# volume-em/empanada-napari

Hardware: AMD Instinct MI355X
Metric: EM tiles/sec (1024^2 fp16) (higher is better)
Workload: dtype f16

## Files before the change

empanada-napari_amd/build.py:

```python
import os
import shutil
import subprocess
import sys

HERE = os.path.dirname(os.path.abspath(__file__))
CSRC = os.path.join(HERE, 'csrc')
OBJ = os.path.join(CSRC, '_obj')
LIBDIR = os.path.join(HERE, 'lib')
LIB = os.path.join(LIBDIR, 'libempanada_hip.so')
ARCH = 'gfx950'

COMMON = ['--offload-arch=' + ARCH, '-O3', '-std=c++17', '-fPIC', '-fvisibility=hidden',
          '-Wall', '-Wno-unused-function', '-Wno-unused-result']
PER_FILE = {
    'postprocess.hip': ['-ffp-contract=off', '-fhip-fp32-correctly-rounded-divide-sqrt'],
}
SOURCES = ['abi.hip', 'conv_igemm.hip', 'layers.hip', 'pointrend.hip', 'postprocess.hip', 'pdl_net.hip', 'sparse.hip',
           'sepconv.hip', 'sepconv_precise.hip', 'conv_igemm256.hip', 'conv_igemm_s64.hip', 'conv3x3c64.hip', 'stem.hip', 'matcher.hip', 'ref32.hip', 'conv16x3.hip', 'conv_igemm_grouped.hip', 'conv16x3p.hip', 'sepconv_x3.hip', 'overlap.hip', 'labels.hip', 'morph.hip']
INCLUDES = {'conv_igemm_grouped.hip': ['conv_igemm.hip']}


def _hipcc():
    for cand in (shutil.which('hipcc'), '/opt/rocm/bin/hipcc'):
        if cand and os.path.exists(cand):
            return cand
    raise RuntimeError('hipcc not found: the HIP engine cannot be built (no CPU fallback exists)')


def _newest_header():
    hs = [os.path.join(CSRC, f) for f in os.listdir(CSRC) if f.endswith('.h')]
    hs.append(os.path.join(HERE, '..', 'include', 'empanada_hip.h'))
    return max(os.path.getmtime(h) for h in hs)


def build_all(verbose=False, force=False):
    os.makedirs(OBJ, exist_ok=True)
    os.makedirs(LIBDIR, exist_ok=True)
    hipcc = _hipcc()
    hdr = _newest_header()
    objs, rebuilt = [], False
    procs = []
    for src in SOURCES:
        s = os.path.join(CSRC, src)
        o = os.path.join(OBJ, src.replace('.hip', '.o'))
        objs.append(o)
        dep = max([os.path.getmtime(s), hdr] + [os.path.getmtime(os.path.join(CSRC, d)) for d in INCLUDES.get(src, [])])
        if force or not os.path.exists(o) or os.path.getmtime(o) < dep:
            cmd = [hipcc] + COMMON + PER_FILE.get(src, []) + ['-c', s, '-o', o]
            if verbose:
                print(' '.join(cmd), flush=True)
            procs.append((src, subprocess.Popen(cmd, stdout=subprocess.PIPE, stderr=subprocess.STDOUT)))
# ... 19 lines not shown
```

empanada-napari_amd/csrc/abi.hip:

```cpp
#include <stdarg.h>

#include <map>
#include <mutex>
#include <utility>
#include <vector>

#include "common.h"

namespace emp {

static thread_local char g_err[1024] = "no error";

void set_error(const char* fmt, ...) {
  va_list ap;
  va_start(ap, fmt);
  vsnprintf(g_err, sizeof(g_err), fmt, ap);
  va_end(ap);
}

const void* zero_page() {
  static void* page = nullptr;
  static std::once_flag once;
  std::call_once(once, [] {
    if (hipMalloc(&page, 2048) != hipSuccess) { page = nullptr; return; }
// ... 83 lines not shown
  p.out = d_out; p.out_ld = out_ld;
  p.N = N; p.H = H; p.W = W; p.Cin = Cin; p.Cout = Cout; p.KH = KH; p.KW = KW; p.stride = stride; p.pad = pad; p.dil = dil;
  p.Ho = (H + 2 * pad - dil * (KH - 1) - 1) / stride + 1;
  p.Wo = (W + 2 * pad - dil * (KW - 1) - 1) / stride + 1;
  EMP_REQUIRE(p.Ho > 0 && p.Wo > 0 && out_ld >= Cout && (d_res == nullptr || res_ld >= Cout), "conv2d_f32: bad output geometry");
  p.act = act;
  return launch_conv32(p, (hipStream_t)stream);
}

int emp_conv2d_nhwc_f16x3(const float* d_in, int N, int H, int W, int Cin, int in_ld, const float* d_w, const float* d_bias,
                          const float* d_bias_n, const float* d_res, int res_ld, float* d_out, int out_ld, int Cout, int KH,
                          int KW, int stride, int pad, int dil, int act, int groups, int cin_g, void* stream) {
  EMP_REQUIRE(d_in && d_w && d_out, "conv2d_f16x3: null pointer");
  EMP_REQUIRE(N > 0 && H > 0 && W > 0 && KH > 0 && KW > 0 && stride > 0 && dil > 0 && pad >= 0 && groups >= 1, "conv2d_f16x3: bad geometry");
  Conv32 p{};
  p.in = d_in; p.in_ld = in_ld; p.w = d_w; p.bias = d_bias; p.bias_n = d_bias_n; p.res = d_res; p.res_ld = res_ld;
  p.out = d_out; p.out_ld = out_ld;
  p.N = N; p.H = H; p.W = W; p.Cin = Cin; p.Cout = Cout; p.KH = KH; p.KW = KW; p.stride = stride; p.pad = pad; p.dil = dil;
  p.Ho = (H + 2 * pad - dil * (KH - 1) - 1) / stride + 1;
  p.Wo = (W + 2 * pad - dil * (KW - 1) - 1) / stride + 1;
  EMP_REQUIRE(p.Ho > 0 && p.Wo > 0 && out_ld >= groups * Cout && (d_res == nullptr || res_ld >= Cout), "conv2d_f16x3: bad output geometry");
  p.act = act;
  p.x3 = 1;
  if (groups > 1) { p.groups = groups; p.cin_g = cin_g; }
  return launch_conv32(p, (hipStream_t)stream);
}

int emp_conv2d_nhwc_f16x3_ex(const float* d_in, int N, int H, int W, int Cin, int in_ld, const float* d_w, const float* d_bias,
                             const float* d_bias_n, const float* d_res, int res_ld, void* d_out, int out_ld, int out_fmt, int Cout, int KH,
                             int KW, int stride, int pad, int dil, int act, int wmode, const float* d_in2, int H2, int W2, int Cin2,
                             int in2_ld, int stride2, const float* d_head_w, const float* d_head_b, int head_c, float* d_head_out,
                             void* stream) {
  EMP_REQUIRE(d_in && d_w && (d_out || d_head_w), "conv2d_f16x3_ex: null pointer");
  EMP_REQUIRE(N > 0 && H > 0 && W > 0 && KH > 0 && KW > 0 && stride > 0 && dil > 0 && pad >= 0 && wmode >= 0 && (wmode & 3) <= 2 && wmode < 8,
              "conv2d_f16x3_ex: bad geometry (wmode 0 fp32 weights, 1 split pairs, 2 pairs + LDS-DMA image; + 4: split-K allowed)");
  const bool ksplit = (wmode & 4) != 0;
  wmode &= 3;
  hipStream_t s = (hipStream_t)stream;
  Conv32 p{};
  p.in = d_in; p.in_ld = in_ld; p.w = d_w; p.bias = d_bias; p.bias_n = d_bias_n; p.res = d_res; p.res_ld = res_ld;
  p.out = (float*)d_out; p.out_ld = out_ld; p.out_fmt = out_fmt;
  p.N = N; p.H = H; p.W = W; p.Cin = Cin; p.Cout = Cout; p.KH = KH; p.KW = KW; p.stride = stride; p.pad = pad; p.dil = dil;
  p.Ho = (H + 2 * pad - dil * (KH - 1) - 1) / stride + 1;
  p.Wo = (W + 2 * pad - dil * (KW - 1) - 1) / stride + 1;
  EMP_REQUIRE(p.Ho > 0 && p.Wo > 0 && (d_head_w || out_ld >= Cout) && (d_res == nullptr || res_ld >= Cout), "conv2d_f16x3_ex: bad output geometry");
  p.act = act;
  p.x3 = 1;
  if (d_in2) { p.in2 = d_in2; p.in2_ld = in2_ld; p.Cin2 = Cin2; p.H2 = H2; p.W2 = W2; p.stride2 = stride2; }
  const int64_t Krow = (int64_t)KH * KW * Cin + (d_in2 ? Cin2 : 0);
  std::vector<void*> tmp;
  auto cleanup = [&]() { for (void* q : tmp) (void)hipFree(q); };
  int rc = EMP_OK;
  if (wmode >= 1) {
    void* d = nullptr;
    if (hipMalloc(&d, (size_t)Cout * Krow * sizeof(uint32_t)) != hipSuccess) { cleanup(); set_error("conv2d_f16x3_ex: out of memory"); return EMP_ERR_NOMEM; }
    tmp.push_back(d);
    p.wpair = (const uint32_t*)d;
    rc = launch_split_pairs(d_w, (uint32_t*)d, (int64_t)Cout * Krow, s);
  }
  if (!rc && wmode == 2 && !d_in2) {
    const int64_t ih = x3_weight_image_halfs(Cout, (int)Krow, Cin);
    if (ih > 0) {
      void* d = nullptr;
      if (hipMalloc(&d, (size_t)ih * sizeof(half_t)) != hipSuccess) { cleanup(); set_error("conv2d_f16x3_ex: out of memory"); return EMP_ERR_NOMEM; }
      tmp.push_back(d);
      p.wimg = (const half_t*)d;
      rc = launch_x3_weight_image(d_w, (half_t*)d, Cout, (int)Krow, s);
    }
  }
  if (!rc && ksplit && !d_head_w && !d_in2) {
    void* d = nullptr;
    if (hipMalloc(&d, (size_t)X3_KPART_BYTES) != hipSuccess) { cleanup(); set_error("conv2d_f16x3_ex: out of memory"); return EMP_ERR_NOMEM; }
    tmp.push_back(d);
    p.kpart = (float*)d; p.kpart_bytes = X3_KPART_BYTES;
  }
  const int64_t MP = (int64_t)N * p.Ho * p.Wo;
  const int tiles = conv16x3_cout_tiles(Cout);
  if (!rc && d_head_w) {
    EMP_REQUIRE(d_head_out && head_c >= 1 && head_c <= 4, "conv2d_f16x3_ex: the fused head writes (N, head_c, Ho * Wo) floats, head_c <= 4");
    void* d = nullptr;
    if (hipMalloc(&d, (size_t)tiles * MP * head_c * sizeof(float)) != hipSuccess) { cleanup(); set_error("conv2d_f16x3_ex: out of memory"); return EMP_ERR_NOMEM; }
    tmp.push_back(d);
    p.head_w = d_head_w; p.head_part = (float*)d; p.head_c = head_c;
    if (!p.out) { p.out = d_head_out; p.out_ld = Cout; }
  }
  if (!rc) rc = launch_conv32(p, s);
  if (!rc && d_head_w) rc = launch_head_finish_f32(p.head_part, tiles, N, p.Ho * p.Wo, head_c, d_head_b, d_head_out, s);
  hipError_t e = hipStreamSynchronize(s);
  cleanup();
  if (!rc && e != hipSuccess) { set_error("conv2d_f16x3_ex: %s", hipGetErrorString(e)); return EMP_ERR_HIP; }
  return rc;
}

int emp_sepconv_x3_pack(const float* d_dw, const float* d_pw, int ks, int C, int Cout, float* d_dw_packed, void* d_pw_packed, void* stream) {
  int rc = launch_sepx3_pack_dw(d_dw, ks, C, C, d_dw_packed, (hipStream_t)stream);
  if (rc) return rc;
  return launch_sepx3_pack_pw(d_pw, C, C, Cout, (half_t*)d_pw_packed, (hipStream_t)stream);
}
int emp_sepconv_x3_nhwc_f32(const float* d_in, int N, int H, int W, int C, int in_ld, const float* d_dw_packed, const void* d_pw_packed,
                            const float* d_bias, int Cout, int act, float* d_out, int out_ld, const float* d_head_w, const float* d_head_b,
// ... 357 lines not shown
```

empanada-napari_amd/csrc/common.h:

```cpp
#pragma once
#include <hip/hip_runtime.h>
#include <stdint.h>
#include <stdio.h>
#include <string>

#include "../../include/empanada_hip.h"

typedef _Float16 half_t;
typedef _Float16 f16x8 __attribute__((ext_vector_type(8)));
typedef _Float16 f16x4 __attribute__((ext_vector_type(4)));
typedef _Float16 f16x2 __attribute__((ext_vector_type(2)));
typedef float f32x4 __attribute__((ext_vector_type(4)));

namespace emp {

void set_error(const char* fmt, ...);

#define EMP_CHECK_HIP(expr)                                                        \
  do {                                                                             \
    hipError_t _e = (expr);                                                        \
    if (_e != hipSuccess) {                                                        \
      emp::set_error("%s:%d: %s -> %s", __FILE__, __LINE__, #expr, hipGetErrorString(_e)); \
      return EMP_ERR_HIP;                                                          \
    }                                                                              \
// ... 94 lines not shown
int launch_sepconvp_pack_pw(const float* w, int pw_ld, int C, int Cout, half_t* packed, hipStream_t s, int wsplit = 0);
int launch_sepconvp_pack_dw(const float* w, int ks, int C, float* packed, hipStream_t s);
int launch_sepconvp(const half_t* in, int N, int H, int W, int C, int in_ld, const float* dww_packed, const half_t* pww_packed,
                    const float* bias, int Cout, int act, half_t* out, int out_ld, const float* head_w,
                    const float* head_b, int head_c, float* hout, int64_t plane, const half_t* zero, hipStream_t s,
                    int ks = 5, int wsplit = 0);
int launch_head1x1(const half_t* in, int N, int P, int K, int in_ld, const float* w, const float* b, int C,
                   float* out, int64_t plane_size, const int32_t* scatter_idx, hipStream_t s);
int launch_bilinear_ac_f32_nchw(const float* in, int NC, int h, int w, float* out, int scale, hipStream_t s);
int launch_zero(void* p, size_t bytes, hipStream_t s);

struct Conv32 {
  const float* in; int in_ld;
  const float* w; const float* bias; const float* bias_n;
  const float* res; int res_ld;
  float* out; int out_ld;
  int N, H, W, Cin, Cout, KH, KW, stride, pad, dil, Ho, Wo;
  int act;
  int ps_cout;
  int groups;
  int cin_g;
  int x3;
  const float* in2; int in2_ld, Cin2, H2, W2, stride2;
  const float* head_w; float* head_part; int head_c;
  int x3_mt, x3_nt, x3_mtx;
  const float* zero;
  const uint32_t* wpair;
  const half_t* wimg;
  int in_fmt, out_fmt, res_fmt;
  const half_t* wimgp;
  float* out2; int out2_ld, split2;
  int x3p_kg;
  float* kpart; int64_t kpart_bytes; int ksplit, x3_ksteps;
};
constexpr int64_t X3_KPART_BYTES = 64ll << 20;
int launch_conv32(const Conv32& p, hipStream_t s);
int launch_conv16x3(const Conv32& p, hipStream_t s);
int launch_split_pairs(const float* w, uint32_t* out, int64_t n, hipStream_t s);
int64_t x3_weight_image_halfs(int Cout, int K, int Cin);
int launch_x3_weight_image(const float* w, half_t* out, int Cout, int K, hipStream_t s);
bool conv16x3p_supported(const Conv32& p);
int launch_conv16x3p(const Conv32& p, hipStream_t s);
int64_t x3p_image_halfs(int Cout, int K);
int x3p_kgroup(int KT, int Cin);
int launch_x3p_pack(const float* w, half_t* out, int Cout, int K, hipStream_t s, int KT = 0, int Cin = 0, int kg = 0);
int launch_hl32_from_f32(const float* in, half_t* out, int64_t rows, int C, int in_ld, int out_ld, hipStream_t s);
int launch_hl32_to_f32(const half_t* in, float* out, int64_t rows, int C, int in_ld, int out_ld, hipStream_t s);
int launch_avgpool_hl32(const half_t* in, int N, int HW, int C, int in_ld, float* out, hipStream_t s);
bool sepconv_x3_supported(int C, int Cout, int head_c, int ks);
int64_t sepx3_pw_halfs(int C, int Cout);
int launch_sepx3_pack_pw(const float* w, int pw_ld, int C, int Cout, half_t* packed, hipStream_t s);
int launch_sepx3_pack_dw(const float* w , int ks, int C, int ld, float* packed, hipStream_t s);
int launch_sepconv_x3(const float* in, int N, int H, int W, int C, int in_ld, const float* dww, const half_t* pww, const float* bias,
                      int Cout, int act, float* out, int out_ld, const float* head_w, const float* head_b, int head_c, float* hout,
                      int64_t plane, hipStream_t s, int ks = 5);
int conv16x3_cout_tiles(int Cout);
int launch_head_finish_f32(const float* part, int tiles, int N, int P, int C, const float* b, float* out, hipStream_t s);
int launch_stem3x3s2_f32(const void* img, int dtype, float sub, float mul, int N, int H, int W, int vh, int vw,
                         const float* w , const float* b, int C, float* out, int out_ld, hipStream_t s);
int launch_gate_mul_f32(float* x, int x_ld, const float* g, int g_ld, int64_t rows, int C, hipStream_t s);
int launch_stem7x7_f32(const void* img, int dtype, float sub, float mul, int N, int H, int W, int vh, int vw,
                       const float* w , const float* b , float* out, hipStream_t s);
int launch_maxpool3x3s2_f32(const float* in, int N, int H, int W, int C, float* out, hipStream_t s);
int launch_dwconv_f32(const float* in, int N, int H, int W, int C, int in_ld, const float* w , int K, float* out,
                      int out_ld, hipStream_t s);
int launch_bilinear_ac_f32_nhwc(const float* in, int N, int h, int w, int C, int in_ld, float* out, int H, int W, int out_ld,
                                hipStream_t s);
int launch_avgpool_f32(const float* in, int N, int HW, int C, int in_ld, float* out, hipStream_t s);
int launch_fuse_combine_f32(const float* a, const float* b, const float* c, float ca, float cb, float cc, int mode, int N,
                            int H, int W, int C, float* out, hipStream_t s);
int launch_head1x1_f32(const float* in, int N, int P, int K, int in_ld, const float* w, const float* b, int C, float* out,
                       int64_t plane_size, const int32_t* scatter_idx, hipStream_t s);
int launch_point_features_f32(const float* feat, int N, int fh, int fw, int C, int feat_ld, const float* coarse, int ncls,
// ... 26 lines not shown
```

empanada-napari_amd/csrc/conv16x3.hip:

```cpp
#include <type_traits>

#include "common.h"

namespace emp {
namespace {

constexpr int X_BK = 32, X_LD = 32;

template <int ACT>
__device__ __forceinline__ float x_act(float x) {
  if (ACT == 1) return fmaxf(x, 0.f);
  if (ACT == 2) return x / (1.f + __expf(-x));
  return x;
}

__device__ __forceinline__ int swz(int r) { return (-((r & 15) >> 2)) & 3; }

__device__ __forceinline__ void lds_barrier() { asm volatile("s_waitcnt lgkmcnt(0)\n\ts_barrier" ::: "memory"); }

__device__ __forceinline__ void split_store(const float4 (&r)[2], half_t* hi, half_t* lo) {
  f16x8 h, l;
#pragma unroll
  for (int q = 0; q < 2; ++q) {
    const float v[4] = {r[q].x, r[q].y, r[q].z, r[q].w};
// ... 649 lines not shown
    if (p.act == 1) hipLaunchKernelGGL(ksplit_finish32_kernel<1>, fg, dim3(256), 0, s, p, total);
    else if (p.act == 2) hipLaunchKernelGGL(ksplit_finish32_kernel<2>, fg, dim3(256), 0, s, p, total);
    else hipLaunchKernelGGL(ksplit_finish32_kernel<0>, fg, dim3(256), 0, s, p, total);
    EMP_LAUNCH_CHECK();
    return EMP_OK;
  }
  if (p.act == 1) return go(&conv16x3s_kernel<1, WPAIR, SLOTS, WIMG>);
  if (p.act == 2) return go(&conv16x3s_kernel<2, WPAIR, SLOTS, WIMG>);
  return go(&conv16x3s_kernel<0, WPAIR, SLOTS, WIMG>);
}

template <int BM, int BN, bool WPAIR, bool DB>
int launch_tile(const Conv32& p, dim3 grid, hipStream_t s) {
  if (p.act == 1) hipLaunchKernelGGL((conv16x3_kernel<1, BM, BN, WPAIR, DB>), grid, dim3(256), 0, s, p);
  else if (p.act == 2) hipLaunchKernelGGL((conv16x3_kernel<2, BM, BN, WPAIR, DB>), grid, dim3(256), 0, s, p);
  else hipLaunchKernelGGL((conv16x3_kernel<0, BM, BN, WPAIR, DB>), grid, dim3(256), 0, s, p);
  EMP_LAUNCH_CHECK();
  return EMP_OK;
}

template <bool WPAIR>
int launch_pair(Conv32 p, hipStream_t s) {
  const int G = p.groups > 1 ? p.groups : 1;
  const int64_t M = (int64_t)p.N * p.Ho * p.Wo;
  const int bn = p.Cout > 64 ? 128 : 64;
  const unsigned nt = (unsigned)((p.Cout + bn - 1) / bn);
  p.x3_mt = (int)((M + 127) / 128);
  p.x3_nt = (int)nt;
  const int kk = p.KH * p.KW * p.Cin;
  static const int rk = [] { const char* e = getenv("EMP_X3_RASTER_K"); return e ? atoi(e) : 64; }();
  p.x3_mtx = (nt >= 2 && kk >= rk) ? (p.x3_mt + 7) / 8 : 0;
  dim3 grid((unsigned)(p.x3_mtx ? 8 * p.x3_mtx * p.x3_nt : p.x3_mt * p.x3_nt), 1u, (unsigned)G);
  static const int kdb = [] { const char* e = getenv("EMP_X3_KDB"); return e ? atoi(e) : 1024; }();
  if (p.head_w) {
    EMP_REQUIRE(p.head_part && p.head_c >= 1 && p.head_c <= 4 && p.act == 1 && G == 1 && !p.res && !p.bias_n && p.ps_cout == 0,
                "conv16x3: fused head needs ReLU, 1..4 head channels, a plain ungrouped convolution");
    if (bn == 128) hipLaunchKernelGGL((conv16x3_kernel<1, 128, 128, WPAIR, false, true>), grid, dim3(256), 0, s, p);
    else hipLaunchKernelGGL((conv16x3_kernel<1, 128, 64, WPAIR, false, true>), grid, dim3(256), 0, s, p);
    EMP_LAUNCH_CHECK();
    return EMP_OK;
  }
  if (p.in2) {
    EMP_REQUIRE(p.act == 1 && bn == 128 && G == 1 && p.ps_cout == 0, "conv16x3: a second source needs ReLU and Cout > 64");
    if (p.KH * p.KW * p.Cin + p.Cin2 >= kdb) hipLaunchKernelGGL((conv16x3_kernel<1, 128, 128, WPAIR, true, false, true>), grid, dim3(256), 0, s, p);
    else hipLaunchKernelGGL((conv16x3_kernel<1, 128, 128, WPAIR, false, false, true>), grid, dim3(256), 0, s, p);
    EMP_LAUNCH_CHECK();
    return EMP_OK;
  }
  const bool db = p.KH * p.KW * p.Cin >= kdb;
  static const int spec = [] { const char* e = getenv("EMP_X3_SPEC"); return e ? atoi(e) : 2; }();
  if (db && spec && bn == 128 && p.Cin % X_BK == 0 && xs_epilogue_ok(p, p.Cout)) {
    static const bool wimg_on = [] { const char* e = getenv("EMP_X3_WIMG"); return !(e && e[0] == '0'); }();
    p.ksplit = 0;
    if (p.kpart && G == 1 && !p.out2 && spec == 2) {
      const int nsteps = kk / X_BK;
      static const int cap = [] { const char* e = getenv("EMP_X3_KSPLIT_WGS"); return e ? atoi(e) : 512; }();
      const int tiles = p.x3_mt * p.x3_nt;
      static const int min_per = [] { const char* e = getenv("EMP_X3_KSPLIT_PER"); return e ? std::max(atoi(e), 4) : 16; }();
      int S = std::min(std::min(8, cap / std::max(tiles, 1)), nsteps / min_per);
      S = S >= 8 ? 8 : (S >= 4 ? 4 : (S >= 2 ? 2 : 0));
      static const int min_steps = [] { const char* e = getenv("EMP_X3_KSPLIT_MINSTEPS"); return e ? atoi(e) : 32; }();
      if (nsteps < min_steps) S = 0;
      if (S >= 2) {
        const int per = (nsteps + S - 1) / S;
        if ((S - 1) * per < nsteps && (int64_t)S * M * p.Cout * 4 <= p.kpart_bytes && ((uintptr_t)p.kpart & 15) == 0) {
          p.ksplit = S; p.x3_ksteps = per;
// ... 115 lines not shown
```

empanada-napari_amd/csrc/pdl_net.hip:

```cpp
#include <string.h>

#include <array>
#include <map>
#include <memory>
#include <string>
#include <vector>

#include "common.h"

namespace emp {

namespace {

struct HostParam {
  std::vector<int64_t> shape;
  std::vector<float> w, b;
  bool set = false;
};

struct Act {
  half_t* p = nullptr;
  int N = 0, H = 0, W = 0, C = 0, ld = 0;
  size_t off = 0;
};
// ... 21 lines not shown
  std::map<std::string, HostParam> params;
  bool finalized = false;
  FILE* layer_log = [] { const char* e = getenv("EMP_LAYER_LOG"); return e ? fopen(e, "w") : (FILE*)nullptr; }();
  bool fuse_stem = [] { const char* e = getenv("EMP_FUSE_STEM"); return !(e && e[0] == '0'); }();
  bool fuse_ds = [] { const char* e = getenv("EMP_FUSE_DS"); return !(e && e[0] == '0'); }();
  bool fuse_b2b = [] { const char* e = getenv("EMP_FUSE_B2B"); return !(e && e[0] == '0'); }();
  bool pack256 = [] { const char* e = getenv("EMP_CONV256_PACK"); return !(e && e[0] == '0'); }();
  bool fuse_proj = [] { const char* e = getenv("EMP_FUSE_PROJ"); return !(e && e[0] == '0'); }();
  bool fuse_aspp = [] { const char* e = getenv("EMP_FUSE_ASPP"); return !(e && e[0] == '0'); }();
  bool fuse_sepconv = [] { const char* e = getenv("EMP_FUSE_SEPCONV"); return !(e && e[0] == '0'); }();
  bool fuse_pr = [] { const char* e = getenv("EMP_FUSE_PR"); return !(e && e[0] == '0'); }();
  int precise_sepconv = [] { const char* e = getenv("EMP_PRECISE_SEPCONV"); return e ? atoi(e) : 1; }();
  bool precise_wsplit = [] { const char* e = getenv("EMP_PRECISE_WSPLIT"); return !(e && e[0] == '0'); }();
  bool precise_fsplit = [] { const char* e = getenv("EMP_PRECISE_FSPLIT"); return !(e && e[0] == '0'); }();
  int sepconv_min_tiles = [] { const char* e = getenv("EMP_SEPCONV_MIN_TILES"); return e ? atoi(e) : 256; }();

  int precision = [] {
    const char* e = getenv("EMP_PRECISION");
    if (e && (!strcmp(e, "fp16") || !strcmp(e, "16"))) return 0;
    if (e && (!strcmp(e, "fp32") || !strcmp(e, "32"))) return 1;
    return 2;
  }();
  bool fp32_graph() const { return precision != 0; }
  bool x3_fuse_ds = [] { const char* e = getenv("EMP_X3_FUSE_DS"); return !(e && e[0] == '0'); }();
  bool x3_fuse_head = [] { const char* e = getenv("EMP_X3_FUSE_HEAD"); return !(e && e[0] == '0'); }();
  bool x3_planes = [] { const char* e = getenv("EMP_X3_PLANES"); return !(e && e[0] == '0'); }();
  int x3_planes_min_tiles = [] { const char* e = getenv("EMP_X3_PLANES_MIN_TILES"); return e ? atoi(e) : 128; }();
  bool x3_planes_ready = false;
  bool x3_ksplit = [] { const char* e = getenv("EMP_X3_KSPLIT"); return !(e && e[0] == '0'); }();
  float* x3_kpart = nullptr;
  bool x3_small_aspp = [] { const char* e = getenv("EMP_X3_SMALL_ASPP"); return !(e && e[0] == '0'); }();
  bool x3_fuse_stem = [] { const char* e = getenv("EMP_X3_FUSE_STEM"); return !(e && e[0] == '0'); }();
  bool x3_merge_proj = [] { const char* e = getenv("EMP_X3_MERGE_PROJ"); return !(e && e[0] == '0'); }();
  bool x3_merge_aspp = [] { const char* e = getenv("EMP_X3_MERGE_ASPP"); return !(e && e[0] == '0'); }();
  bool x3_fuse_sep = [] { const char* e = getenv("EMP_X3_FUSE_SEP"); return !(e && e[0] == '0'); }();
  int x3_sep_min_tiles = [] { const char* e = getenv("EMP_X3_SEP_MIN_TILES"); return e ? atoi(e) : 1; }();
  struct SepX3 { float* dw = nullptr; half_t* pw = nullptr; int C = 0, Cout = 0, ks = 0; };
  std::map<std::string, SepX3> sepx3;
  bool regnet_grouped = [] { const char* e = getenv("EMP_REGNET_GROUPED"); return !(e && e[0] == '0'); }();
  int64_t regnet_group_tiles = [] { const char* e = getenv("EMP_REGNET_GROUP_TILES"); return e ? atoll(e) : 2048ll; }();
  struct W32 { float* w = nullptr; float* b = nullptr; int cout = 0, cin = 0, cin16 = 0, kh = 1, kw = 1; uint32_t* wp = nullptr; int cin2 = 0, cin2_16 = 0; half_t* wimg = nullptr; half_t* wimgp = nullptr; int x3p_kg = 0; };
  std::map<std::string, W32> w32;
  std::map<std::string, std::pair<float*, size_t>> pool32;
  std::map<std::string, std::array<int, 4>> geom32;

  std::map<std::string, DevConv> convs;
  std::map<std::string, float*> f32w;
  std::map<std::string, half_t*> f16w;
  std::map<std::string, std::vector<float>> fusew;
  std::vector<void*> owned;

  char* arena = nullptr;
  size_t arena_cap = 0, arena_used = 0;
  int pN = 0, pH = 0, pW = 0, pRS = 0;
  int capN = 0;
  std::map<std::string, Act> acts;
  std::vector<std::string> act_order;
  std::map<std::string, std::pair<size_t, size_t>> raw;
  double flops = 0.0;
  size_t image_bytes = 0;
  bool profile = false;
  std::vector<std::pair<hipEvent_t, hipEvent_t>> prof_events;
  size_t prof_used = 0;
  double prof_flops = 0.0;
  int64_t par_limit = [] { const char* e = getenv("EMP_PAR_DECODERS"); return e ? atoll(e) : (int64_t)4 << 20; }();
  hipStream_t aux = nullptr;
  hipEvent_t ev_fork = nullptr, ev_join = nullptr;

  ~emp_pdl() {
    for (void* p : owned) (void)hipFree(p);
    for (auto& kv : pool32) (void)hipFree(kv.second.first);
    if (arena) (void)hipFree(arena);
    if (layer_log) fclose(layer_log);
    for (auto& e : prof_events) { (void)hipEventDestroy(e.first); (void)hipEventDestroy(e.second); }
// ... 1290 lines not shown
    for (auto& kv : n->w32) {
      const std::string& nm = kv.first;
      if (nm.size() < 10 || nm.compare(nm.size() - 10, 10, ".sepconv.1") != 0) continue;
      const std::string base = nm.substr(0, nm.size() - 2);
      auto dwi = n->f32w.find(base + ".0.dw32");
      auto hpi = n->params.find(base + ".0");
      if (dwi == n->f32w.end() || hpi == n->params.end() || hpi->second.shape.size() != 4) continue;
      const emp_pdl::W32& w = kv.second;
      const int ks = (int)hpi->second.shape[2], C = w.cin16;
      if (w.kh != 1 || w.kw != 1 || !sepconv_x3_supported(C, w.cout, 0, ks)) continue;
      emp_pdl::SepX3 sx;
      sx.C = C; sx.Cout = w.cout; sx.ks = ks;
      void* d = nullptr;
      EMP_CHECK_HIP(hipMalloc(&d, (size_t)ks * ks * C * sizeof(float)));
      n->owned.push_back(d);
      sx.dw = (float*)d;
      RC32(launch_sepx3_pack_dw(dwi->second, ks, C, C, sx.dw, nullptr));
      EMP_CHECK_HIP(hipMalloc(&d, (size_t)sepx3_pw_halfs(C, w.cout) * sizeof(half_t)));
      n->owned.push_back(d);
      sx.pw = (half_t*)d;
      RC32(launch_sepx3_pack_pw(w.w, C, C, w.cout, sx.pw, nullptr));
      n->sepx3[base] = sx;
    }
    EMP_CHECK_HIP(hipStreamSynchronize(nullptr));
  }
  if (n->precision == 2 && c.arch == 0 && c.ins_decoder && n->x3_merge_proj) {
    for (int i = 0; i < c.n_stages; ++i) {
      const std::string a = "semantic_decoder.project." + std::to_string(i) + ".0", b = "instance_decoder.project." + std::to_string(i) + ".0";
      auto ia = n->w32.find(a), ib = n->w32.find(b);
      if (ia == n->w32.end() || ib == n->w32.end()) continue;
      const emp_pdl::W32 &wa = ia->second, &wb = ib->second;
      if (wa.cin16 != wb.cin16 || wa.kh != 1 || wb.kh != 1 || wa.kw != 1 || wb.kw != 1 || wa.cout % 4 || wb.cout % 4 || wa.cin16 >= 1024) continue;
      emp_pdl::W32 m = wa;
      m.cout = wa.cout + wb.cout; m.wp = nullptr; m.wimg = nullptr; m.wimgp = nullptr;
      const size_t na = (size_t)wa.cout * wa.cin16, nb = (size_t)wb.cout * wb.cin16;
      void* d = nullptr;
      EMP_CHECK_HIP(hipMalloc(&d, (na + nb) * sizeof(float)));
      n->owned.push_back(d);
      m.w = (float*)d;
      EMP_CHECK_HIP(hipMemcpy(m.w, wa.w, na * sizeof(float), hipMemcpyDeviceToDevice));
      EMP_CHECK_HIP(hipMemcpy(m.w + na, wb.w, nb * sizeof(float), hipMemcpyDeviceToDevice));
      EMP_CHECK_HIP(hipMalloc(&d, (size_t)m.cout * sizeof(float)));
      n->owned.push_back(d);
      m.b = (float*)d;
      EMP_CHECK_HIP(hipMemcpy(m.b, wa.b, (size_t)wa.cout * sizeof(float), hipMemcpyDeviceToDevice));
      EMP_CHECK_HIP(hipMemcpy(m.b + wa.cout, wb.b, (size_t)wb.cout * sizeof(float), hipMemcpyDeviceToDevice));
      n->w32["decoders.project." + std::to_string(i) + ".0"] = m;
    }
  }
  if (n->precision == 2) {
    for (auto& kv : n->w32) {
      emp_pdl::W32& w = kv.second;
      const int64_t cnt = (int64_t)w.cout * (w.kh * w.kw * w.cin16 + w.cin2_16);
      void* d = nullptr;
      EMP_CHECK_HIP(hipMalloc(&d, (size_t)(cnt > 0 ? cnt : 4) * sizeof(uint32_t)));
      n->owned.push_back(d);
      w.wp = (uint32_t*)d;
      RC32(launch_split_pairs(w.w, w.wp, cnt, nullptr));
      const int K = w.kh * w.kw * w.cin16;
      const int64_t ih = (w.cin2_16 == 0 && K >= 1024) ? x3_weight_image_halfs(w.cout, K, w.cin16) : 0;
      if (ih > 0) {
        EMP_CHECK_HIP(hipMalloc(&d, (size_t)ih * sizeof(half_t)));
        n->owned.push_back(d);
        w.wimg = (half_t*)d;
        RC32(launch_x3_weight_image(w.w, w.wimg, w.cout, K, nullptr));
      }
      const bool region = kv.first.find("encoder.layer3.") == 0 || kv.first.find("encoder.layer4.") == 0 || kv.first.find(".aspp.") != std::string::npos;
      const int64_t ip = (n->x3_planes && n->cfg.encoder == 0 && region && w.cin2_16 == 0 && w.cin16 % 32 == 0 && K >= 128) ? x3p_image_halfs(w.cout, K) : 0;
      if (ip > 0) {
        EMP_CHECK_HIP(hipMalloc(&d, (size_t)ip * sizeof(half_t)));
        n->owned.push_back(d);
        w.wimgp = (half_t*)d;
        w.x3p_kg = x3p_kgroup(w.kh * w.kw, w.cin16);
        RC32(launch_x3p_pack(w.w, w.wimgp, w.cout, K, nullptr, w.kh * w.kw, w.cin16, w.x3p_kg));
      }
    }
    if (n->x3_planes && c.encoder == 0 && c.arch == 0 && c.ins_decoder && n->x3_merge_aspp) {
      for (int i = 0; i <= 3; ++i) {
        const std::string a = "semantic_decoder.aspp.convs." + std::to_string(i) + ".0", b = "instance_decoder.aspp.convs." + std::to_string(i) + ".0";
        auto ia = n->w32.find(a), ib = n->w32.find(b);
        if (ia == n->w32.end() || ib == n->w32.end()) continue;
        const emp_pdl::W32 &wa = ia->second, &wb = ib->second;
        if (!wa.wimgp || !wb.wimgp || wa.cout != wb.cout || wa.cin16 != wb.cin16 || wa.kh != wb.kh || wa.kw != wb.kw) continue;
        emp_pdl::W32 m = wa;
        m.cout = wa.cout + wb.cout; m.wp = nullptr; m.wimg = nullptr; m.wimgp = nullptr;
        const size_t K = (size_t)wa.kh * wa.kw * wa.cin16, na = (size_t)wa.cout * K, nb = (size_t)wb.cout * K;
        void* d = nullptr;
        EMP_CHECK_HIP(hipMalloc(&d, (na + nb) * sizeof(float)));
        n->owned.push_back(d);
        m.w = (float*)d;
        EMP_CHECK_HIP(hipMemcpy(m.w, wa.w, na * sizeof(float), hipMemcpyDeviceToDevice));
        EMP_CHECK_HIP(hipMemcpy(m.w + na, wb.w, nb * sizeof(float), hipMemcpyDeviceToDevice));
        EMP_CHECK_HIP(hipMalloc(&d, (size_t)m.cout * sizeof(float)));
        n->owned.push_back(d);
        m.b = (float*)d;
        EMP_CHECK_HIP(hipMemcpy(m.b, wa.b, (size_t)wa.cout * sizeof(float), hipMemcpyDeviceToDevice));
        EMP_CHECK_HIP(hipMemcpy(m.b + wa.cout, wb.b, (size_t)wb.cout * sizeof(float), hipMemcpyDeviceToDevice));
        const int64_t ip = x3p_image_halfs(m.cout, (int)K);
        if (ip <= 0) continue;
        EMP_CHECK_HIP(hipMalloc(&d, (size_t)ip * sizeof(half_t)));
        n->owned.push_back(d);
        m.wimgp = (half_t*)d;
        m.x3p_kg = x3p_kgroup(m.kh * m.kw, m.cin16);
        RC32(launch_x3p_pack(m.w, m.wimgp, m.cout, (int)K, nullptr, m.kh * m.kw, m.cin16, m.x3p_kg));
        n->w32["decoders.aspp.convs." + std::to_string(i) + ".0"] = m;
      }
    }
    EMP_CHECK_HIP(hipStreamSynchronize(nullptr));
    if (n->x3_planes && c.encoder == 0) {
      bool ok = true;
      for (auto& kv : n->w32) {
        const bool region = kv.first.find("encoder.layer3.") == 0 || kv.first.find("encoder.layer4.") == 0 || kv.first.find(".aspp.") != std::string::npos;
        const bool boundary = kv.first == "encoder.layer3.0.conv1" || kv.first == "encoder.layer3.0.downsample.0" || kv.first.find("conv3+ds") != std::string::npos;
        if (region && !boundary && !kv.second.wimgp) ok = false;
      }
      for (int i = 0; i < (c.arch == 0 ? c.n_stages : 0); ++i) ok = ok && c.low_level_stages[i] <= 2;
      n->x3_planes_ready = ok;
    }
// ... 3 lines not shown

int c32(emp_pdl* n, const std::string& wname, const T32& in, int in_coff, const T32& out, int out_coff, int stride, int pad,
        int dil, int act, const T32* res, const float* bias_n, hipStream_t s, int ps_cout = 0, int groups = 1,
        const float* head_w = nullptr, float* head_part = nullptr, int head_c = 0, const T32* in2 = nullptr, int stride2 = 1,
        const T32* out2 = nullptr, int out2_coff = 0, int split2 = 0) {
  const emp_pdl::W32& w = n->w32.at(wname);
  Conv32 p{};
  if (out2) {
    EMP_REQUIRE(n->precision == 2 && out2->fmt == out.fmt && (!out2->fmt || out2_coff % 32 == 0) && (in.fmt || !out.fmt), "%s: bad second destination", wname.c_str());
    p.out2 = out2->p + out2_coff; p.out2_ld = out2->ld; p.split2 = split2;
  }
  if (groups > 1) {
    EMP_REQUIRE(w.cout % groups == 0 && in_coff == 0 && out_coff == 0 && !res && !bias_n && !ps_cout, "%s (fp32): bad grouped call",
                wname.c_str());
    p.groups = groups;
    p.cin_g = w.cin;
  }
  EMP_REQUIRE((!in.fmt || in_coff % 32 == 0) && (!out.fmt || out_coff % 32 == 0), "%s: hl32 channel slices start at multiples of 32", wname.c_str());
  EMP_REQUIRE(!in.fmt || (w.wimgp && groups <= 1 && !in2 && !head_w && !ps_cout), "%s: an hl32 input needs the packed image of a plain convolution", wname.c_str());
  p.in = in.p + in_coff; p.in_ld = in.ld; p.in_fmt = in.fmt;
  p.wimgp = in.fmt ? w.wimgp : nullptr;
  p.x3p_kg = w.x3p_kg;
  p.w = w.w; p.bias = w.b; p.bias_n = bias_n;
  p.res = res ? res->p : nullptr; p.res_ld = res ? res->ld : 0; p.res_fmt = res ? res->fmt : 0;
  p.out = out.p + out_coff; p.out_ld = out.ld; p.out_fmt = out.fmt;
  p.N = in.N; p.H = in.H; p.W = in.W; p.Cin = w.cin16; p.Cout = w.cout / groups; p.KH = w.kh; p.KW = w.kw;
  p.stride = stride; p.pad = pad; p.dil = dil;
  p.Ho = (in.H + 2 * pad - dil * (w.kh - 1) - 1) / stride + 1;
  p.Wo = (in.W + 2 * pad - dil * (w.kw - 1) - 1) / stride + 1;
  p.act = act; p.ps_cout = ps_cout;
  p.x3 = n->precision == 2;
  p.wpair = p.x3 ? w.wp : nullptr;
  p.wimg = (p.x3 && groups <= 1) ? w.wimg : nullptr;
  p.head_w = head_w; p.head_part = head_part; p.head_c = head_c;
  if (p.x3 && n->x3_ksplit && n->x3_kpart && !head_w && !in2 && (in.fmt || !out2)) { p.kpart = n->x3_kpart; p.kpart_bytes = X3_KPART_BYTES; }
  if (in2) {
    EMP_REQUIRE(p.x3 && w.cin2_16 > 0 && w.cin2_16 <= in2->ld && in2->N == in.N, "%s: second source mismatch", wname.c_str());
    p.in2 = in2->p; p.in2_ld = in2->ld; p.Cin2 = w.cin2_16; p.H2 = in2->H; p.W2 = in2->W; p.stride2 = stride2;
    n->flops += 2.0 * (double)p.N * p.Ho * p.Wo * w.cout * (double)w.cin2;
  } else {
    EMP_REQUIRE(w.cin2_16 == 0, "%s: packed for two sources", wname.c_str());
  }
  EMP_REQUIRE(!head_w || p.x3, "%s: the fused head exists in the fp16x3 mode only", wname.c_str());
  const int up = ps_cout ? 2 : 1;
  EMP_REQUIRE(p.Ho * up == out.H && p.Wo * up == out.W && in.N == out.N, "%s (fp32): output shape mismatch", wname.c_str());
  EMP_REQUIRE(in_coff + (groups - 1) * w.cin + w.cin16 <= in.ld && out_coff + (ps_cout ? ps_cout : (out2 ? split2 : w.cout)) <= out.ld,
              "%s (fp32): channel slice out of range (needs %d of a row of %d)", wname.c_str(), in_coff + (groups - 1) * w.cin + w.cin16, in.ld);
  n->flops += 2.0 * (double)p.N * p.Ho * p.Wo * w.cout * (double)(w.cin * w.kh * w.kw);
  if (n->profile && p.x3 && p.in_fmt) {
    if (n->prof_used == n->prof_events.size()) {
      hipEvent_t a, b;
      EMP_CHECK_HIP(hipEventCreate(&a));
      EMP_CHECK_HIP(hipEventCreate(&b));
      n->prof_events.emplace_back(a, b);
    }
    auto& ev = n->prof_events[n->prof_used++];
    EMP_CHECK_HIP(hipEventRecord(ev.first, s));
    const int rc = launch_conv32(p, s);
    EMP_CHECK_HIP(hipEventRecord(ev.second, s));
    n->prof_flops += 3.0 * 2.0 * (double)p.N * p.Ho * p.Wo * w.cout * (double)(w.cin16 * w.kh * w.kw);
    return rc;
  }
  return launch_conv32(p, s);
}

int run32(emp_pdl* n, const void* img, int dtype, float sub, float mul, int N, int H, int W, int vh, int vw, int RS, int interp,
// ... 896 lines not shown
```

Baseline: 1371.

## Add register-resident-weight persistent kernel for 1x1 ReLU expansion convolutions

Adds a specialized fp16x3 kernel for 1x1 stride-1 ReLU expansion convolutions (Cin 64->256, 128->512). Each wave keeps its split hi/lo weights in registers for the whole run, and persistent workgroups loop over 128-row tiles, prefetching the next tile's input and the residual while running MFMAs. A pre-split weight image is built at load time and the path is on by default once there are at least 128 tiles. The goal is to cut the repeated weight traffic and generic-kernel overhead of these bottleneck expansions, at the cost of extra weight memory and a narrowly scoped code path.

```diff
diff --git a/empanada-napari_amd/build.py b/empanada-napari_amd/build.py
--- a/empanada-napari_amd/build.py
+++ b/empanada-napari_amd/build.py
@@ -16,7 +16,7 @@
     'postprocess.hip': ['-ffp-contract=off', '-fhip-fp32-correctly-rounded-divide-sqrt'],
 }
 SOURCES = ['abi.hip', 'conv_igemm.hip', 'layers.hip', 'pointrend.hip', 'postprocess.hip', 'pdl_net.hip', 'sparse.hip',
-           'sepconv.hip', 'sepconv_precise.hip', 'conv_igemm256.hip', 'conv_igemm_s64.hip', 'conv3x3c64.hip', 'stem.hip', 'matcher.hip', 'ref32.hip', 'conv16x3.hip', 'conv_igemm_grouped.hip', 'conv16x3p.hip', 'sepconv_x3.hip', 'overlap.hip', 'labels.hip', 'morph.hip']
+           'sepconv.hip', 'sepconv_precise.hip', 'conv_igemm256.hip', 'conv_igemm_s64.hip', 'conv3x3c64.hip', 'stem.hip', 'matcher.hip', 'ref32.hip', 'conv16x3.hip', 'conv16x3e.hip', 'conv_igemm_grouped.hip', 'conv16x3p.hip', 'sepconv_x3.hip', 'overlap.hip', 'labels.hip', 'morph.hip']
 INCLUDES = {'conv_igemm_grouped.hip': ['conv_igemm.hip']}
 
 
diff --git a/empanada-napari_amd/csrc/abi.hip b/empanada-napari_amd/csrc/abi.hip
--- a/empanada-napari_amd/csrc/abi.hip
+++ b/empanada-napari_amd/csrc/abi.hip
@@ -139,10 +139,11 @@
                              int in2_ld, int stride2, const float* d_head_w, const float* d_head_b, int head_c, float* d_head_out,
                              void* stream) {
   EMP_REQUIRE(d_in && d_w && (d_out || d_head_w), "conv2d_f16x3_ex: null pointer");
-  EMP_REQUIRE(N > 0 && H > 0 && W > 0 && KH > 0 && KW > 0 && stride > 0 && dil > 0 && pad >= 0 && wmode >= 0 && (wmode & 3) <= 2 && wmode < 8,
-              "conv2d_f16x3_ex: bad geometry (wmode 0 fp32 weights, 1 split pairs, 2 pairs + LDS-DMA image; + 4: split-K allowed)");
-  const bool ksplit = (wmode & 4) != 0;
+  EMP_REQUIRE(N > 0 && H > 0 && W > 0 && KH > 0 && KW > 0 && stride > 0 && dil > 0 && pad >= 0 && wmode >= 0 && (wmode & 3) <= 2 && wmode < 16,
+              "conv2d_f16x3_ex: bad geometry (wmode 0 fp32 weights, 1 split pairs, 2 pairs + LDS-DMA image; + 4: split-K allowed; + 8: the expansion kernel or an error)");
+  const bool ksplit = (wmode & 4) != 0, expand = (wmode & 8) != 0;
   wmode &= 3;
+  EMP_REQUIRE(!expand || wmode >= 1, "conv2d_f16x3_ex: the expansion kernel (wmode | 8) reads pre-split weights: wmode 1 or 2, not fp32 weights");
   hipStream_t s = (hipStream_t)stream;
   Conv32 p{};
   p.in = d_in; p.in_ld = in_ld; p.w = d_w; p.bias = d_bias; p.bias_n = d_bias_n; p.res = d_res; p.res_ld = res_ld;
@@ -173,6 +174,17 @@
       tmp.push_back(d);
       p.wimg = (const half_t*)d;
       rc = launch_x3_weight_image(d_w, (half_t*)d, Cout, (int)Krow, s);
+    }
+  }
+  if (!rc && expand) {
+    p.x3e = 2;
+    const int64_t ih = d_in2 ? 0 : x3e_image_halfs(Cout, (int)Krow, Cin);
+    if (ih > 0) {
+      void* d = nullptr;
+      if (hipMalloc(&d, (size_t)ih * sizeof(half_t)) != hipSuccess) { cleanup(); set_error("conv2d_f16x3_ex: out of memory"); return EMP_ERR_NOMEM; }
+      tmp.push_back(d);
+      p.wimge = (const half_t*)d;
+      rc = launch_x3e_weight_image(d_w, (half_t*)d, Cout, (int)Krow, s);
     }
   }
   if (!rc && ksplit && !d_head_w && !d_in2) {
diff --git a/empanada-napari_amd/csrc/common.h b/empanada-napari_amd/csrc/common.h
--- a/empanada-napari_amd/csrc/common.h
+++ b/empanada-napari_amd/csrc/common.h
@@ -150,6 +150,7 @@
   float* out2; int out2_ld, split2;
   int x3p_kg;
   float* kpart; int64_t kpart_bytes; int ksplit, x3_ksteps;
+  const half_t* wimge; int x3e, x3e_min_tiles;
 };
 constexpr int64_t X3_KPART_BYTES = 64ll << 20;
 int launch_conv32(const Conv32& p, hipStream_t s);
@@ -157,6 +158,10 @@
 int launch_split_pairs(const float* w, uint32_t* out, int64_t n, hipStream_t s);
 int64_t x3_weight_image_halfs(int Cout, int K, int Cin);
 int launch_x3_weight_image(const float* w, half_t* out, int Cout, int K, hipStream_t s);
+bool conv16x3e_supported(const Conv32& p);
+int launch_conv16x3e(const Conv32& p, hipStream_t s);
+int64_t x3e_image_halfs(int Cout, int K, int Cin);
+int launch_x3e_weight_image(const float* w, half_t* out, int Cout, int K, hipStream_t s);
 bool conv16x3p_supported(const Conv32& p);
 int launch_conv16x3p(const Conv32& p, hipStream_t s);
 int64_t x3p_image_halfs(int Cout, int K);
diff --git a/empanada-napari_amd/csrc/conv16x3.hip b/empanada-napari_amd/csrc/conv16x3.hip
--- a/empanada-napari_amd/csrc/conv16x3.hip
+++ b/empanada-napari_amd/csrc/conv16x3.hip
@@ -705,6 +705,12 @@
   p.x3_mtx = (nt >= 2 && kk >= rk) ? (p.x3_mt + 7) / 8 : 0;
   dim3 grid((unsigned)(p.x3_mtx ? 8 * p.x3_mtx * p.x3_nt : p.x3_mt * p.x3_nt), 1u, (unsigned)G);
   static const int kdb = [] { const char* e = getenv("EMP_X3_KDB"); return e ? atoi(e) : 1024; }();
+  if (p.x3e) {
+    const bool ok = conv16x3e_supported(p);
+    EMP_REQUIRE(ok || p.x3e != 2, "conv16x3: the expansion kernel takes a 1x1 stride-1 ReLU convolution of one fp32 source, Cin 64 -> Cout 256 or 128 -> 512, with its weight image (got %dx%d stride %d, Cin %d -> Cout %d, act %d)",
+                p.KH, p.KW, p.stride, p.Cin, p.Cout, p.act);
+    if (ok && (p.x3e == 2 || p.x3_mt >= p.x3e_min_tiles)) return launch_conv16x3e(p, s);
+  }
   if (p.head_w) {
     EMP_REQUIRE(p.head_part && p.head_c >= 1 && p.head_c <= 4 && p.act == 1 && G == 1 && !p.res && !p.bias_n && p.ps_cout == 0,
                 "conv16x3: fused head needs ReLU, 1..4 head channels, a plain ungrouped convolution");
diff --git a/empanada-napari_amd/csrc/conv16x3e.hip b/empanada-napari_amd/csrc/conv16x3e.hip
--- /dev/null
+++ b/empanada-napari_amd/csrc/conv16x3e.hip
@@ -0,0 +1,225 @@
+#include <stdlib.h>
+
+#include <algorithm>
+
+#include "common.h"
+
+namespace emp {
+namespace {
+
+constexpr int E_BM = 128;
+constexpr int E_LD = 32;
+constexpr int E_TILE = E_BM * E_LD;
+constexpr int E_TLD = 68;
+
+__device__ __forceinline__ int swz(int r) { return (-((r & 15) >> 2)) & 3; }
+__device__ __forceinline__ void lds_barrier() { asm volatile("s_waitcnt lgkmcnt(0)\n\ts_barrier" ::: "memory"); }
+__device__ __forceinline__ void split_store4(const float4& r, half_t* hi, half_t* lo) {
+  const float v[4] = {r.x, r.y, r.z, r.w};
+  f16x4 h, l;
+#pragma unroll
+  for (int e = 0; e < 4; ++e) {
+    const half_t a = (half_t)v[e];
+    h[e] = a;
+    l[e] = (half_t)(v[e] - (float)a);
+  }
+  *reinterpret_cast<f16x4*>(hi) = h;
+  *reinterpret_cast<f16x4*>(lo) = l;
+}
+
+constexpr int x3e_lds_bytes(int KS, int NW, int NJ) { return KS * 2 * E_TILE * 2 + NW * 16 * NJ * E_TLD * 4; }
+
+template <int KS, int NW, int NJ, bool BN>
+__global__ void __launch_bounds__(NW * 64, 2) conv16x3e_kernel(const Conv32 p, const int ntiles) {
+  constexpr int RP = NW * 8;
+  constexpr int NP = E_BM / RP;
+  constexpr int NX = NP * KS;
+  constexpr int NG = E_BM / (16 * NJ);
+  constexpr int NQ = 4 * NJ;
+  static_assert(NG % 2 == 0, "the residual register sets alternate: group 0 of every tile reads set 0");
+  extern __shared__ __attribute__((aligned(1024))) char e_lds[];
+  half_t* const Xh = reinterpret_cast<half_t*>(e_lds);
+  half_t* const Xl = Xh + KS * E_TILE;
+  const int tid = threadIdx.x, lane = tid & 63;
+  const int wave = __builtin_amdgcn_readfirstlane(tid >> 6);
+  float* const Tr = reinterpret_cast<float*>(Xl + KS * E_TILE) + wave * (16 * NJ * E_TLD);
+  const int HoWo = p.Ho * p.Wo;
+  const int M = p.N * HoWo;
+  f16x8 wh[KS][4], wl[KS][4];
+  {
+    const f16x8* wi = reinterpret_cast<const f16x8*>(p.wimge) + (size_t)wave * (KS * 4 * 2 * 64) + lane;
+#pragma unroll
+    for (int ks = 0; ks < KS; ++ks)
+#pragma unroll
+      for (int i = 0; i < 4; ++i) {
+        wh[ks][i] = wi[((ks * 4 + i) * 2 + 0) * 64];
+        wl[ks][i] = wi[((ks * 4 + i) * 2 + 1) * 64];
+      }
+  }
+  const int srow = tid >> 3, sc4 = tid & 7;
+  const int soff = srow * E_LD + ((((sc4 >> 1) ^ swz(srow)) << 3) | ((sc4 & 1) << 2));
+  float4 rx[NX];
+  auto xload = [&](int tile, int x) {
+    const int ks = x / NP, pp = x % NP;
+    const int row = srow + RP * pp;
+    const bool ok = tile < ntiles && tile * E_BM + row < M;
+    const float* src = ok ? p.in + (size_t)(tile * E_BM + row) * p.in_ld + ks * 32 + sc4 * 4 : p.zero;
+    rx[x] = *reinterpret_cast<const float4*>(src);
+  };
+  const int ep = lane >> 4, ec = (lane & 15) * 4;
+  const int co = wave * 64 + ec;
+  const float4 bi = p.bias ? *reinterpret_cast<const float4*>(p.bias + co) : make_float4(0.f, 0.f, 0.f, 0.f);
+  float4 rr[2][NQ];
+  auto rload = [&](int m0, int g, int set) {
+#pragma unroll
+    for (int q = 0; q < NQ; ++q) {
+      const int m = m0 + g * 16 * NJ + q * 4 + ep;
+      const float* src = (p.res && m < M) ? p.res + (size_t)m * p.res_ld + co : p.zero;
+      rr[set][q] = *reinterpret_cast<const float4*>(src);
+    }
+  };
+  const int fr = lane & 15, fq = lane >> 4;
+  const int foff = fr * E_LD + ((fq ^ swz(fr)) << 3);
+
+  auto group = [&](int m0, int g, int set) {
+    f32x4 acc[4][NJ];
+#pragma unroll
+    for (int i = 0; i < 4; ++i)
+#pragma unroll
+      for (int j = 0; j < NJ; ++j) acc[i][j] = f32x4{0.f, 0.f, 0.f, 0.f};
+#pragma unroll
+    for (int ks = 0; ks < KS; ++ks) {
+#pragma unroll
+      for (int j = 0; j < NJ; ++j) {
+        const int xo = ks * E_TILE + (g * 16 * NJ + j * 16) * E_LD + foff;
+        const f16x8 xh = *reinterpret_cast<const f16x8*>(Xh + xo);
+        const f16x8 xl = *reinterpret_cast<const f16x8*>(Xl + xo);
+#pragma unroll
+        for (int i = 0; i < 4; ++i) acc[i][j] = __builtin_amdgcn_mfma_f32_16x16x32_f16(wl[ks][i], xh, acc[i][j], 0, 0, 0);
+#pragma unroll
+        for (int i = 0; i < 4; ++i) acc[i][j] = __builtin_amdgcn_mfma_f32_16x16x32_f16(wh[ks][i], xh, acc[i][j], 0, 0, 0);
+#pragma unroll
+        for (int i = 0; i < 4; ++i) acc[i][j] = __builtin_amdgcn_mfma_f32_16x16x32_f16(wh[ks][i], xl, acc[i][j], 0, 0, 0);
+      }
+    }
+#pragma unroll
+    for (int j = 0; j < NJ; ++j)
+#pragma unroll
+      for (int i = 0; i < 4; ++i) *reinterpret_cast<f32x4*>(Tr + (j * 16 + fr) * E_TLD + i * 16 + fq * 4) = acc[i][j];
+    __builtin_amdgcn_wave_barrier();
+#pragma unroll
+    for (int q = 0; q < NQ; ++q) {
+      const int m = m0 + g * 16 * NJ + q * 4 + ep;
+      const f32x4 a = *reinterpret_cast<const f32x4*>(Tr + (q * 4 + ep) * E_TLD + ec);
+      float4 t = make_float4(a[0] + bi.x, a[1] + bi.y, a[2] + bi.z, a[3] + bi.w);
+      if (BN && m < M) {
+        const float4 b = *reinterpret_cast<const float4*>(p.bias_n + (size_t)(m / HoWo) * p.Cout + co);
+        t.x += b.x; t.y += b.y; t.z += b.z; t.w += b.w;
+      }
+      if (p.res) {
+        const float4 r = rr[set][q];
+        t.x += r.x; t.y += r.y; t.z += r.z; t.w += r.w;
+      }
+      if (m < M)
+        *reinterpret_cast<float4*>(p.out + (size_t)m * p.out_ld + co) = make_float4(fmaxf(t.x, 0.f), fmaxf(t.y, 0.f), fmaxf(t.z, 0.f), fmaxf(t.w, 0.f));
+    }
+    __builtin_amdgcn_wave_barrier();
+  };
+
+  int tile = blockIdx.x;
+#pragma unroll
+  for (int x = 0; x < NX; ++x) xload(tile, x);
+  for (; tile < ntiles; tile += (int)gridDim.x) {
+    const int m0 = tile * E_BM;
+    lds_barrier();
+#pragma unroll
+    for (int x = 0; x < NX; ++x) {
+      const int o = (x / NP) * E_TILE + soff + (x % NP) * RP * E_LD;
+      split_store4(rx[x], Xh + o, Xl + o);
+    }
+    rload(m0, 0, 0);
+    lds_barrier();
+    const int nxt = tile + (int)gridDim.x;
+#pragma unroll
+    for (int g = 0; g < NG; ++g) {
+      if (g + 1 < NG) rload(m0, g + 1, (g + 1) & 1);
+#pragma unroll
+      for (int x = 0; x < NX; ++x)
+        if (x * (NG - 1) / NX == g) xload(nxt, x);
+      group(m0, g, g & 1);
+    }
+  }
+}
+
+__global__ void __launch_bounds__(256) x3e_weight_image_kernel(const float* __restrict__ w, half_t* __restrict__ out, int Cout, int K) {
+  const int KS = K / 32;
+  const int64_t total = (int64_t)(Cout / 64) * KS * 4 * 64;
+  for (int64_t t = (int64_t)blockIdx.x * 256 + threadIdx.x; t < total; t += (int64_t)gridDim.x * 256) {
+    const int lane = (int)(t & 63), i = (int)((t >> 6) & 3);
+    const int64_t wk = t >> 8;
+    const int ks = (int)(wk % KS), wv = (int)(wk / KS);
+    const int cout = wv * 64 + i * 16 + (lane & 15), k0 = ks * 32 + (lane >> 4) * 8;
+    f16x8 h, l;
+#pragma unroll
+    for (int e = 0; e < 8; ++e) {
+      const float x = w[(size_t)cout * K + k0 + e];
+      const half_t a = (half_t)x;
+      h[e] = a;
+      l[e] = (half_t)(x - (float)a);
+    }
+    half_t* base = out + ((size_t)((wk * 4 + i) * 2) * 64 + lane) * 8;
+    *reinterpret_cast<f16x8*>(base) = h;
+    *reinterpret_cast<f16x8*>(base + 64 * 8) = l;
+  }
+}
+
+template <int KS, int NW, int NJ, bool BN>
+int launch_e(const Conv32& p, int ntiles, int cus, int cap, hipStream_t s) {
+  constexpr int LDS = x3e_lds_bytes(KS, NW, NJ);
+  static_assert(LDS <= 160 * 1024, "LDS of one workgroup");
+  auto kern = &conv16x3e_kernel<KS, NW, NJ, BN>;
+  if (int rc = ensure_dyn_lds(reinterpret_cast<const void*>(kern), LDS)) return rc;
+  const int per_cu = std::min(160 * 1024 / LDS, 16 / NW);
+  const int grid = std::max(1, std::min(ntiles, cap > 0 ? cap : cus * per_cu));
+  hipLaunchKernelGGL(kern, dim3((unsigned)grid), dim3(NW * 64), LDS, s, p, ntiles);
+  EMP_LAUNCH_CHECK();
+  return EMP_OK;
+}
+
+}
+
+bool conv16x3e_shape_ok(int Cin, int Cout) { return (Cin == 64 || Cin == 128) && Cout == 4 * Cin; }
+
+bool conv16x3e_supported(const Conv32& p) {
+  return p.wimge && conv16x3e_shape_ok(p.Cin, p.Cout) && p.KH == 1 && p.KW == 1 && p.stride == 1 && p.pad == 0 && p.act == 1 && p.groups <= 1 &&
+         !p.in2 && !p.head_w && !p.out2 && p.ps_cout == 0 && p.in_fmt == 0 && p.out_fmt == 0 && p.res_fmt == 0 && p.H == p.Ho && p.W == p.Wo &&
+         p.in_ld >= p.Cin && p.out_ld >= p.Cout && (!p.res || p.res_ld >= p.Cout) && (p.in_ld & 3) == 0 && (((uintptr_t)p.in) & 15) == 0 && (((uintptr_t)p.wimge) & 15) == 0 && (p.out_ld & 3) == 0 &&
+         (((uintptr_t)p.out) & 15) == 0 && (!p.bias || (((uintptr_t)p.bias) & 15) == 0) && (!p.bias_n || (((uintptr_t)p.bias_n) & 15) == 0) &&
+         (!p.res || ((p.res_ld & 3) == 0 && (((uintptr_t)p.res) & 15) == 0)) && (int64_t)p.N * p.Ho * p.Wo + E_BM < (1ll << 31);
+}
+
+int launch_conv16x3e(const Conv32& p, hipStream_t s) {
+  EMP_REQUIRE(conv16x3e_supported(p) && p.zero, "conv16x3e: unsupported launch");
+  static const int cus = [] {
+    int dev = 0, n = 0;
+    if (hipGetDevice(&dev) != hipSuccess || hipDeviceGetAttribute(&n, hipDeviceAttributeMultiprocessorCount, dev) != hipSuccess || n <= 0) n = 256;
+    return n;
+  }();
+  const char* e = getenv("EMP_X3_EXPAND_WGS");
+  const int cap = e ? atoi(e) : 0;
+  const int ntiles = (int)(((int64_t)p.N * p.Ho * p.Wo + E_BM - 1) / E_BM);
+  if (p.bias_n) return p.Cin == 64 ? launch_e<2, 4, 2, true>(p, ntiles, cus, cap, s) : launch_e<4, 8, 1, true>(p, ntiles, cus, cap, s);
+  return p.Cin == 64 ? launch_e<2, 4, 2, false>(p, ntiles, cus, cap, s) : launch_e<4, 8, 1, false>(p, ntiles, cus, cap, s);
+}
+
+int64_t x3e_image_halfs(int Cout, int K, int Cin) { return (K == Cin && conv16x3e_shape_ok(Cin, Cout)) ? 2ll * Cout * K : 0; }
+
+int launch_x3e_weight_image(const float* w, half_t* out, int Cout, int K, hipStream_t s) {
+  EMP_REQUIRE(w && out && conv16x3e_shape_ok(K, Cout), "x3e_weight_image: bad shape");
+  const int64_t total = (int64_t)(Cout / 64) * (K / 32) * 256;
+  hipLaunchKernelGGL(x3e_weight_image_kernel, dim3((unsigned)((total + 255) / 256)), dim3(256), 0, s, w, out, Cout, K);
+  EMP_LAUNCH_CHECK();
+  return EMP_OK;
+}
+
+}
diff --git a/empanada-napari_amd/csrc/pdl_net.hip b/empanada-napari_amd/csrc/pdl_net.hip
--- a/empanada-napari_amd/csrc/pdl_net.hip
+++ b/empanada-napari_amd/csrc/pdl_net.hip
@@ -77,6 +77,8 @@
   bool x3_small_aspp = [] { const char* e = getenv("EMP_X3_SMALL_ASPP"); return !(e && e[0] == '0'); }();
   bool x3_fuse_stem = [] { const char* e = getenv("EMP_X3_FUSE_STEM"); return !(e && e[0] == '0'); }();
   bool x3_merge_proj = [] { const char* e = getenv("EMP_X3_MERGE_PROJ"); return !(e && e[0] == '0'); }();
+  bool x3_expand = [] { const char* e = getenv("EMP_X3_EXPAND"); return !(e && e[0] == '0'); }();
+  int x3_expand_min_tiles = [] { const char* e = getenv("EMP_X3_EXPAND_MIN_TILES"); return e ? atoi(e) : 128; }();
   bool x3_merge_aspp = [] { const char* e = getenv("EMP_X3_MERGE_ASPP"); return !(e && e[0] == '0'); }();
   bool x3_fuse_sep = [] { const char* e = getenv("EMP_X3_FUSE_SEP"); return !(e && e[0] == '0'); }();
   int x3_sep_min_tiles = [] { const char* e = getenv("EMP_X3_SEP_MIN_TILES"); return e ? atoi(e) : 1; }();
@@ -84,7 +86,7 @@
   std::map<std::string, SepX3> sepx3;
   bool regnet_grouped = [] { const char* e = getenv("EMP_REGNET_GROUPED"); return !(e && e[0] == '0'); }();
   int64_t regnet_group_tiles = [] { const char* e = getenv("EMP_REGNET_GROUP_TILES"); return e ? atoll(e) : 2048ll; }();
-  struct W32 { float* w = nullptr; float* b = nullptr; int cout = 0, cin = 0, cin16 = 0, kh = 1, kw = 1; uint32_t* wp = nullptr; int cin2 = 0, cin2_16 = 0; half_t* wimg = nullptr; half_t* wimgp = nullptr; int x3p_kg = 0; };
+  struct W32 { float* w = nullptr; float* b = nullptr; int cout = 0, cin = 0, cin16 = 0, kh = 1, kw = 1; uint32_t* wp = nullptr; int cin2 = 0, cin2_16 = 0; half_t* wimg = nullptr; half_t* wimgp = nullptr; int x3p_kg = 0; half_t* wimge = nullptr; };
   std::map<std::string, W32> w32;
   std::map<std::string, std::pair<float*, size_t>> pool32;
   std::map<std::string, std::array<int, 4>> geom32;
@@ -1441,7 +1443,7 @@
       const emp_pdl::W32 &wa = ia->second, &wb = ib->second;
       if (wa.cin16 != wb.cin16 || wa.kh != 1 || wb.kh != 1 || wa.kw != 1 || wb.kw != 1 || wa.cout % 4 || wb.cout % 4 || wa.cin16 >= 1024) continue;
       emp_pdl::W32 m = wa;
-      m.cout = wa.cout + wb.cout; m.wp = nullptr; m.wimg = nullptr; m.wimgp = nullptr;
+      m.cout = wa.cout + wb.cout; m.wp = nullptr; m.wimg = nullptr; m.wimgp = nullptr; m.wimge = nullptr;
       const size_t na = (size_t)wa.cout * wa.cin16, nb = (size_t)wb.cout * wb.cin16;
       void* d = nullptr;
       EMP_CHECK_HIP(hipMalloc(&d, (na + nb) * sizeof(float)));
@@ -1474,6 +1476,13 @@
         w.wimg = (half_t*)d;
         RC32(launch_x3_weight_image(w.w, w.wimg, w.cout, K, nullptr));
       }
+      const int64_t ie = (n->x3_expand && w.cin2_16 == 0 && w.kh == 1 && w.kw == 1) ? x3e_image_halfs(w.cout, K, w.cin16) : 0;
+      if (ie > 0) {
+        EMP_CHECK_HIP(hipMalloc(&d, (size_t)ie * sizeof(half_t)));
+        n->owned.push_back(d);
+        w.wimge = (half_t*)d;
+        RC32(launch_x3e_weight_image(w.w, w.wimge, w.cout, K, nullptr));
+      }
       const bool region = kv.first.find("encoder.layer3.") == 0 || kv.first.find("encoder.layer4.") == 0 || kv.first.find(".aspp.") != std::string::npos;
       const int64_t ip = (n->x3_planes && n->cfg.encoder == 0 && region && w.cin2_16 == 0 && w.cin16 % 32 == 0 && K >= 128) ? x3p_image_halfs(w.cout, K) : 0;
       if (ip > 0) {
@@ -1492,7 +1501,7 @@
         const emp_pdl::W32 &wa = ia->second, &wb = ib->second;
         if (!wa.wimgp || !wb.wimgp || wa.cout != wb.cout || wa.cin16 != wb.cin16 || wa.kh != wb.kh || wa.kw != wb.kw) continue;
         emp_pdl::W32 m = wa;
-        m.cout = wa.cout + wb.cout; m.wp = nullptr; m.wimg = nullptr; m.wimgp = nullptr;
+        m.cout = wa.cout + wb.cout; m.wp = nullptr; m.wimg = nullptr; m.wimgp = nullptr; m.wimge = nullptr;
         const size_t K = (size_t)wa.kh * wa.kw * wa.cin16, na = (size_t)wa.cout * K, nb = (size_t)wb.cout * K;
         void* d = nullptr;
         EMP_CHECK_HIP(hipMalloc(&d, (na + nb) * sizeof(float)));
@@ -1562,6 +1571,7 @@
   p.x3 = n->precision == 2;
   p.wpair = p.x3 ? w.wp : nullptr;
   p.wimg = (p.x3 && groups <= 1) ? w.wimg : nullptr;
+  if (p.x3 && groups <= 1 && w.wimge && act == 1 && stride == 1) { p.wimge = w.wimge; p.x3e = 1; p.x3e_min_tiles = n->x3_expand_min_tiles; }
   p.head_w = head_w; p.head_part = head_part; p.head_c = head_c;
   if (p.x3 && n->x3_ksplit && n->x3_kpart && !head_w && !in2 && (in.fmt || !out2)) { p.kpart = n->x3_kpart; p.kpart_bytes = X3_KPART_BYTES; }
   if (in2) {
```

Result: no change. 1376, median of 4 (+0.4%).
